# Nilau1998/SAC-Agent

Measured on AMD Instinct MI355X. Metric: env-steps/sec (whole node), boat_env exp-6, 65 536 envs/GPU at 1/2/4/8 MI355X, higher is better.
Workload: dtype f64

## Files before the change

sac-agent_amd/csrc/sacenv_boat.hip:

```cpp

#include <hip/hip_runtime.h>
#include <stdint.h>
#include <string.h>

#include "sacenv.h"

#pragma clang fp contract(off)

namespace {

constexpr int kWave = 64;
constexpr int kMtN = SACENV_MT_N;
constexpr int kMtM = 397;
constexpr uint32_t kMtUpper = 0x80000000u;
constexpr uint32_t kMtLower = 0x7fffffffu;
constexpr uint32_t kMtMatrixA = 0x9908b0dfu;
constexpr int kMaxK = SACENV_MAX_KNOTS;
constexpr int kSlots = SACENV_SLOTS;
constexpr double kPi = 3.141592653589793;

constexpr int U_SX = 0, U_SY = 8, U_SR = 16, U_VX = 24, U_VY = 32, U_VR = 40, U_RUD = 48,
              U_EP = 56, U_COEF = 64, U_W0N = 128, U_T = 144, U_IDX = 152,
              U_CONS = 156, U_FILL = 160, U_MTPOS = 164, U_SYN = 168, U_STARTY = 172,
              U_CNT = U_STARTY + 4 * kSlots,
// ... 320 lines not shown
#pragma unroll
  for (int i = 4; i < 10; ++i) ps = fma_v(ps, z, K.s[i]);
  double pc = fma_v(z, K.c[0], K.c[1]);
#pragma unroll
  for (int i = 2; i < 7; ++i) pc = fma_v(pc, z, K.c[i]);
  sincos_quadrant(r, z, ps, pc, k, sp, cp);
}

__device__ __forceinline__ void sincos_quadrant(double r, double z, double ps, double pc, double k, double* sp,
                                                double* cp) {
  const double sr = fma(r * z, ps, r);
  const double cr = 1.0 - fma(-(z * z), pc, 0.5 * z);
  const int q = (int)k;
  const double a = (q & 1) ? cr : sr, b = (q & 1) ? sr : cr;
  const uint64_t ms = (uint64_t)(((uint32_t)q << 30) & 0x80000000u) << 32;
  const uint64_t mc = (uint64_t)((((uint32_t)q + 1u) << 30) & 0x80000000u) << 32;
  *sp = __longlong_as_double((long long)((uint64_t)__double_as_longlong(a) ^ ms));
  *cp = __longlong_as_double((long long)((uint64_t)__double_as_longlong(b) ^ mc));
}

struct SinCos {
  double s, c;
};
__device__ __forceinline__ double sin_ocml(double x) { return sin(x); }
__device__ __forceinline__ SinCos sincos_ocml(double x) {
  SinCos r;
  sincos(x, &r.s, &r.c);
  return r;
}

__device__ __forceinline__ void sincos_cw(double x, double* sp, double* cp, const TrigK& K) {
  sincos_fast(x, sp, cp, K);
  const bool ok = fabs(x) <= kCwBound;
  if (__ballot(!ok) != 0ull && !ok) {
    const SinCos r = sincos_ocml(x);
    *sp = r.s, *cp = r.c;
  }
}

__device__ __forceinline__ void trig3(double j, double r, double w, double* sj, double* sr, double* sw,
                                      double* cw, const TrigK& K) {
  const double kw = rint(w * 0.6366197723675814);
  double rw = fma(-kw, 1.5707963267948966, w);
  rw = fma(-kw, 6.123233995736766e-17, rw);
  rw = fma(-kw, -1.4973849048591698e-33, rw);
  const double zj = j * j, zr = r * r, zw = rw * rw;
  double qj = fma_v(zj, K.s[0], K.s[1]);
  double qr = fma_v(zr, K.s[0], K.s[1]);
  double ps = 0.0, pc = 0.0;
#pragma unroll
  for (int i = 2; i < 10; ++i) {
    qj = fma_v(qj, zj, K.s[i]);
    qr = fma_v(qr, zr, K.s[i]);
    if (i == 3) ps = fma_v(zw, K.s[2], K.s[3]);
    if (i >= 4) ps = fma_v(ps, zw, K.s[i]);
    if (i == 4) pc = fma_v(zw, K.c[0], K.c[1]);
    if (i >= 5) pc = fma_v(pc, zw, K.c[i - 3]);
  }
  *sj = fma(j * zj, qj, j);
  *sr = fma(r * zr, qr, r);
  sincos_quadrant(rw, zw, ps, pc, kw, sw, cw);
  const bool okj = fabs(j) <= kSinBound, okr = fabs(r) <= kSinBound, okw = fabs(w) <= kCwBound;
  if (__ballot(!(okj && okr && okw)) != 0ull) {
    if (!okj) *sj = sin_ocml(j);
    if (!okr) *sr = sin_ocml(r);
    if (!okw) {
      const SinCos q = sincos_ocml(w);
      *sw = q.s, *cw = q.c;
    }
  }
}

__device__ __forceinline__ double div_c(double x, double c, double r) {
  const double q = x * r;
  const double err = fma(-q, c, x);
  return fma(err, r, q);
}

struct Obs {
  float v[SACENV_OBS_DIM];
};

struct ObsConst {
  double goal, two_w, fuel;
  double k[8];
};

__device__ __forceinline__ ObsConst obs_const(const Tail& T) {
  return ObsConst{T.r_goal, T.r_two_w, T.r_fuel,
                  {1.0 / 5.0, 1.0 / 0.025, 1.0 / 0.37, 1.0 / (2 * kPi), 1.0 / 8.5e-3, 1.0 / 1.4e-5,
                   1.0 / (kPi / 3 - (-kPi / 3)), kPi / 3}};
}
__device__ __forceinline__ ObsConst obs_const_v(const Tail& T) {
  ObsConst o = obs_const(T);
#pragma unroll
  for (int i = 0; i < 8; ++i) o.k[i] = vconst(o.k[i]);
// ... 1097 lines not shown
  int64_t act_stride;
  const uint32_t* ready;
  uint32_t* done;
  uint32_t seq0;
  int32_t* status;
};

__device__ __forceinline__ uint32_t flag_issue(const uint32_t* f) {
  const __amdgpu_buffer_rsrc_t r =
      __builtin_amdgcn_make_buffer_rsrc(const_cast<uint32_t*>(f), 0, 4, 0x00020000);
  return __builtin_amdgcn_raw_buffer_load_b32(r, 0, 0, 17);
}
__device__ __forceinline__ uint32_t flag_value(uint32_t v) {
  return (uint32_t)__builtin_amdgcn_readfirstlane((int)v);
}
__device__ __forceinline__ uint32_t flag_load(const uint32_t* f) { return flag_value(flag_issue(f)); }
__device__ __forceinline__ float act_load(const char* row, uint32_t off) {
  const __amdgpu_buffer_rsrc_t r = __builtin_amdgcn_make_buffer_rsrc(const_cast<char*>(row), 0, 0x7fffffff,
                                                                     0x00020000);
  return __builtin_bit_cast(float, __builtin_amdgcn_raw_buffer_load_b32(r, off, 0, 17));
}
__device__ uint32_t wait_flag(const uint32_t* f, uint32_t want, uint32_t seen, int32_t* status, int lane) {
  for (uint32_t it = 0; seen < want; ++it) {
    if (it >= kSpinLimit) {
      if (lane == 0) atomicOr(status, SACENV_STATUS_HANDOFF_TIMEOUT);
      return 0u;
    }
    __builtin_amdgcn_s_sleep(2);
    seen = flag_load(f);
  }
  return seen;
}

template <bool kRoll, int kNc, bool kTIdx, bool kHand = false, int kRows = 1, bool kVc = kRoll>
__device__ __forceinline__ void owner_wave(const SacenvBoatParams& pin, const Arena& A, const Tail& Tin,
                                           const float* __restrict__ action, OwnerLds& l, int ob,
                                           int lane, int n_steps = 1, const RollArgs* ra = nullptr,
                                           char* trans1 = nullptr, uint32_t seen0 = 0u) {
#ifdef SACENV_STAMPS
  const uint64_t st_real0 = __builtin_amdgcn_s_memrealtime();
  uint64_t st_loaded = 0, st_computed = 0;
#define OWNER_STAMP(v)                                            \
  do {                                                            \
    if (!kRoll) {    \
      asm volatile("s_waitcnt vmcnt(0) lgkmcnt(0)" ::: "memory"); \
      v = __builtin_amdgcn_s_memrealtime();                       \
    }                                                             \
  } while (0)
#else
#define OWNER_STAMP(v) \
  do {                 \
  } while (0)
#endif
  const int e = ob * kWave + lane;
  const uint32_t eo = (uint32_t)e * 8u, eo4 = (uint32_t)e * 4u;
  const char* const wbase = A.wk_wave(ob * kWave);
  const bool active = e < pin.n_envs;
  const char* const abase = reinterpret_cast<const char*>(action) + (active ? eo4 : (uint32_t)ob * 256u);
  uint32_t lt = (uint32_t)A.i32e(U_LTERM, eo4);
  const uint32_t* const rdy = kHand ? (ra->ready != nullptr ? ra->ready + ob : nullptr) : nullptr;
  const int64_t arow = kRoll ? ra->act_stride * 4 : 0;
  uint32_t seen = seen0;
  bool failed = false;
  const bool per_step = kHand && rdy != nullptr && seen < ra->seq0 + (uint32_t)n_steps;
  float act_cur = *reinterpret_cast<const float*>(abase);
  constexpr bool t_idx = kTIdx;
  constexpr int nc = kNc;
  int32_t index = A.i32e(U_IDX, eo4);
  int cons = pin.autoreset ? A.i32e(U_CONS, eo4) : 0;
  double cf[kCoef];
#pragma unroll
  for (int k = 0; k < kCoef; ++k) cf[k] = 0.0;
  if (nc > 0) {
#pragma unroll
    for (int k = 0; k < 4; k += 2) {
      const double2 q = A.f64p(U_COEF + 8 * k, eo);
      cf[k] = q.x, cf[k + 1] = q.y;
    }
    if (nc > 1) {
#pragma unroll
      for (int k = 4; k < 8; k += 2) {
        const double2 q = A.f64p(U_COEF + 8 * k, eo);
        cf[k] = q.x, cf[k + 1] = q.y;
      }
    }
  }
  const double2 p_sxy = A.f64p(U_SX, eo), p_srvx = A.f64p(U_SR, eo), p_vyvr = A.f64p(U_VY, eo);
  const double2 p_rudep = A.f64p(U_RUD, eo);
  double s_x = p_sxy.x, s_y = p_sxy.y, s_r = p_srvx.x;
  double v_x = p_srvx.y, v_y = p_vyvr.x, v_r = p_vyvr.y;
  double rudder = p_rudep.x, t = t_idx ? 0.0 : A.f64e(U_T, eo), ep = p_rudep.y;
  __builtin_amdgcn_sched_barrier(0);
  const SacenvBoatParams& p = pin;
  const Tail& T = Tin;
  constexpr bool kWT = !kRoll || kHand;
  const TrigK K = trig_k<kVc>();
  const ObsConst oc = kVc ? obs_const_v(T) : obs_const(T);
  double y0c[2] = {0.0, 0.0};
  int32_t syc = 0;
  if (kRoll && p.autoreset) {
#pragma unroll
    for (int c = 0; c < 2; ++c)
      if (c < nc) y0c[c] = A.f64e(U_W0N + 8 * c, eo);
    if (p.experiment == 2) syc = A.i32e(U_SYN, eo4);
  }
#ifdef SACENV_STAMPS
  uint64_t ph[4] = {0, 0, 0, 0}, ph_t = 0;
#define PHASE(i)                                         \
  do {                                                   \
    __builtin_amdgcn_sched_barrier(0);                   \
    const uint64_t ph_now = __builtin_amdgcn_s_memtime(); \
    if ((i) > 0) ph[(i) - 1] += ph_now - ph_t;           \
    ph_t = ph_now;                                       \
    __builtin_amdgcn_sched_barrier(0);                   \
  } while (0)
#else
#define PHASE(i) \
  do {           \
  } while (0)
#endif
  Knot kcur = knot_coord(p, index > p.wind_len - 1 ? p.wind_len - 1 : index);
  const uint32_t slot_bytes = 2u * 16u * (uint32_t)A.nk, lane_ring = A.wko_l(0, 0, 0, lane);
  const int slot0 = cons % kSlots;
  int nslot = slot0 + 1 == kSlots ? 0 : slot0 + 1;
  uint32_t so = lane_ring + (uint32_t)slot0 * slot_bytes, sno = lane_ring + (uint32_t)nslot * slot_bytes;
  if (kRoll && kRows == 2) {
    static_assert((kMkWords & (kMkWords - 1)) == 0, "l.mk is indexed (ks / 32) % kMkWords");
    if (ra->marks != nullptr) {
      const int W = (n_steps + 63) / 64;
      unsigned long long* const w = ra->marks + (int64_t)e * W;
      for (int q = 0; q < W; ++q) {
        const unsigned long long m = w[q];
        w[q] = 0ull;
        l.mk[2 * q][lane] = (uint32_t)m;
        l.mk[2 * q + 1][lane] = (uint32_t)(m >> 32);
      }
    } else {
#pragma unroll
      for (int q = 0; q < kMkWords; ++q) l.mk[q][lane] = ~0u;
    }
    __builtin_amdgcn_fence(__ATOMIC_RELEASE, "wavefront");
    __builtin_amdgcn_wave_barrier();
    __builtin_amdgcn_fence(__ATOMIC_ACQUIRE, "wavefront");
  }
  const __amdgpu_buffer_rsrc_t srs = __builtin_amdgcn_make_buffer_rsrc(
      (kRoll && kRows == 2) ? ra->stage + (int64_t)ob * kWave * n_steps * 64 : nullptr, 0, 0x7fffffff, 0x00020000);
  const uint32_t s_lane = (kRoll && kRows == 2) ? (uint32_t)lane * (uint32_t)n_steps * 64u : 0u;
  uint32_t mkw = 0u;
  if (kRoll) __builtin_amdgcn_s_waitcnt(0);
  for (int ks = 0; ks < (kRoll ? n_steps : 1) && (!kHand || !failed); ++ks) {
  PHASE(0);
  const float act = active ? act_cur : 0.0f;
  bool act_next = false;
  uint32_t flag_now = 0u;
  if (kRoll && ks + 1 < n_steps) {
    if (!kHand || !per_step) {
      act_cur = *reinterpret_cast<const float*>(abase + (int64_t)(ks + 1) * arow);
      act_next = true;
    } else {
      if (seen >= ra->seq0 + (uint32_t)ks + 2u) {
        act_cur = act_load(abase, (uint32_t)((ks + 1) * arow));
        act_next = true;
      }
      flag_now = flag_issue(rdy);
    }
  }
  const int wi = index > p.wind_len - 1 ? p.wind_len - 1 : index;
  Knot knext = kcur;
  double wv = 0.0, wa = 0.0;
  bool refresh = false;
  int jn = 0;
  double rq[kCoef];
  if (nc == 0) {
    wind_at(p, A, T.table, 0, e, wi, wv, wa);
  } else {
    const double tt = kcur.t;
    const double c0 = spline_piece(cf[0], cf[2], cf[1], cf[3], tt);
    if (nc == 2) {
      wv = c0;
      wa = spline_piece(cf[4], cf[6], cf[5], cf[7], tt);
    } else if (p.experiment == 4) {
      wv = c0;
      wa = p.wind_dir_rad;
    } else {
      wv = p.max_velocity;
      wa = ((c0 <= 0.5 / 2 ? 0.0 : 1.0) * kPi) + kPi / 2;
    }
    const int wn = index + 1 > p.wind_len - 1 ? p.wind_len - 1 : index + 1;
    knext = knot_coord(p, wn);
    jn = knext.j;
    refresh = index == 0 || jn != kcur.j;
    if (__ballot(refresh) != 0ull) {
#pragma unroll
      for (int c = 0; c < 2; ++c)
        if (c < nc) {
          double q[4];
          A.piece_at(wbase, refresh ? so + (uint32_t)(c * A.nk + jn) * 16u : 0u, q);
          rq[4 * c] = q[0], rq[4 * c + 1] = q[1], rq[4 * c + 2] = q[2], rq[4 * c + 3] = q[3];
        }
    }
  }
  double y0n[2];
  int32_t syn = 0;
  const bool hdr_refresh = p.autoreset && index == 0;
  {
    const int ns = nslot;
#pragma unroll
    for (int c = 0; c < 2; ++c)
      if (c < nc) {
        const double v = *(hdr_refresh ? reinterpret_cast<const double*>(wbase + sno + (uint32_t)(c * A.nk) * 16u)
                                       : (kRoll ? A.wind_knots() : &A.f64e(U_W0N + 8 * c, eo)));
        y0n[c] = kRoll && !hdr_refresh ? y0c[c] : v;
      }
    if (nc == 0 && p.experiment == 2) {
      const int32_t v = *(hdr_refresh ? &A.i32e(U_STARTY + 4 * ns, eo4) : &A.i32e(U_SYN, eo4));
      syn = kRoll && !hdr_refresh ? syc : v;
    }
  }
  OWNER_STAMP(st_loaded);
  const double r_mx = T.r_mx, r_my = T.r_my, r_iz = T.r_iz, r_nd = T.r_nd, r_w = T.r_w;

  t = t_idx ? (double)(index + 1) * p.dt : t + p.dt;
  const int32_t fuel = p.fuel0 - (index + 1);
  if (p.test_mode == 0) rudder = rudder + div_c((double)act, 10.0, 0.1);
  if (!t_idx) EARLY_STORE(U_T, t);
  const bool first = index == 0;
  const double v_x_w = v_x * p.one_minus_wf;
  const double J = p.n_rpm != 0.0 ? div_c(v_x_w, p.n_times_d, r_nd) : 0.0;
  double sin_J, sin_rud, swa, cwa;
  trig3(J, rudder, wa, &sin_J, &sin_rud, &swa, &cwa, K);
  PHASE(1);

  const double F_R = (v_x * v_x) * T.k_front;
  const double F_T = sin_J * T.k_thrust;
  const double F_C = v_y * p.m_plus_my * v_r;
  const double w2s = wv * fabs(wv);
  const double F_W = (w2s * T.k_front) * cwa;
  const double a_x = div_c(-F_R + F_T + F_C + F_W, p.m_plus_mx, r_mx);
  v_x = first ? 3.0 : a_x * p.dt + v_x;

  const double F_R2 = (v_y * fabs(v_y)) * T.k_side;
  const double vx2 = v_x * v_x;
  const double F_RU = sin_rud * (vx2 * T.k_rud_front);
  const double F_C2 = v_x * p.m_plus_mx * v_r;
  const double F_W2 = (w2s * T.k_side) * swa;
  const double a_y = div_c(-F_R2 + F_RU + F_C2 + F_W2, p.m_plus_my, r_my);
  v_y = first ? 0.0 : a_y * p.dt + v_y;
// ... 3 lines not shown
  const double a_r = div_c(-M_hull + M_rud, p.i_plus_iz, r_iz);
  v_r = first ? 0.0 : a_r * p.dt + v_r;
  EARLY_STORE2(U_VY, v_y, v_r);

  s_r = v_r * p.dt + s_r;
  double ssr, csr;
  sincos_cw(s_r, &ssr, &csr, K);
  s_x = (v_x * csr - v_y * ssr) * p.dt + s_x;
  s_y = (v_y * csr + v_x * ssr) * p.dt + s_y;
  index = index + 1;
  EARLY_STORE2(U_SX, s_x, s_y);
  EARLY_STORE2(U_SR, s_r, v_x);
  if (!kRoll) st_out(A.i32e(U_IDX, eo4), index);
  PHASE(2);

  Obs o = make_obs(p, oc, s_x, v_x, a_x, s_y, v_y, a_y, s_r, v_r, a_r, rudder, (double)fuel);

  const double ay = fabs(s_y);
  const double f_y = div_c(ay, p.track_width, r_w) / (1.0 + exp_v(p.reward_k * (ay - p.reward_center), K));
  double reward = 0.0 - f_y;

  const bool goal = s_x >= p.goal_line;
  int tm = (rudder > kPi / 3) | (rudder < -kPi / 3) ? SACENV_TERM_RUDDER_BROKEN : SACENV_TERM_NONE;
  tm = p.t_max <= t ? SACENV_TERM_TIMEOUT : tm;
  tm = fuel < 0 ? SACENV_TERM_OUT_OF_FUEL : tm;
  tm = (fabs(s_y) > p.oob_limit) | (s_x < 0.0) ? SACENV_TERM_OUT_OF_BOUNDS : tm;
  tm = goal ? SACENV_TERM_REACHED_GOAL : tm;
  reward = goal ? reward + 1000.0 : reward;
  reward = ((rudder > kPi / 4) | (rudder < -kPi / 4)) ? reward - fabs(rudder) * 100.0 : reward;
  reward = fabs(s_r) > kPi / 2 ? reward - 1.0 : reward;
  ep = ep + reward;
  uint8_t term = active ? (uint8_t)tm : (uint8_t)SACENV_TERM_NONE;

  if (term != SACENV_TERM_NONE)
    __hip_atomic_fetch_add(&A.at_e<uint32_t>(U_CNT + 4 * (term - 1), eo4), 1u, __ATOMIC_RELAXED,
                           __HIP_MEMORY_SCOPE_AGENT);
  if (term == SACENV_TERM_NONE && active && p.max_episode_steps > 0 && index >= p.max_episode_steps)
    term = SACENV_TERM_TRUNCATED;
  lt = (uint32_t)term - 1u < 5u ? (uint32_t)term : lt;
  const bool ended = term != SACENV_TERM_NONE;
  PHASE(3);

  OWNER_STAMP(st_computed);
  char* const R = kRoll ? ra->rec + (int64_t)ks * ra->rec_stride : A.b + A.ur() * A.np;
  float* const fin = kRoll ? (ra->fin != nullptr ? ra->fin + (int64_t)ks * ra->fin_stride : nullptr)
                           : A.final_obs();
  char* const trans = kRows != 1 ? nullptr
                              : kRoll ? (ra->trans != nullptr ? ra->trans + (int64_t)ks * ra->trans_stride : nullptr)
                                      : trans1;
  if (p.out_flags & SACENV_OUT_REWARD64) A.at_e<double>(A.ur() + 126, eo) = reward;
  if (p.out_flags & SACENV_OUT_ACCEL) {
    A.at_e<double>(A.ur() + 102, eo) = a_x;
    A.at_e<double>(A.ur() + 110, eo) = a_y;
    A.at_e<double>(A.ur() + 118, eo) = a_r;
  }
  const bool restart = ended && p.autoreset;
  if (ended) A.at_e<double>(A.ur() + 94, eo) = ep;
  if (restart && fin != nullptr) store_obs(fin + (int64_t)e * SACENV_OBS_DIM, o);
  int cons_out = cons;
  bool staged = false;
  if (kRoll && kRows == 2) {
    if ((ks & 31) == 0) mkw = l.mk[(ks >> 5) & (kMkWords - 1)][lane];
    staged = (mkw & 1u) != 0u;
    mkw >>= 1;
    if (staged) {
      const uint32_t so = (uint32_t)ks * 64u;
      __builtin_amdgcn_raw_buffer_store_b128(
          u4v{__float_as_uint(o.v[0]), __float_as_uint(o.v[1]), __float_as_uint(o.v[2]), __float_as_uint(o.v[3])},
          srs, s_lane, so, 0);
      __builtin_amdgcn_raw_buffer_store_b128(
          u4v{__float_as_uint(o.v[4]), __float_as_uint(o.v[5]), __float_as_uint(o.v[6]), __float_as_uint(o.v[7])},
          srs, s_lane + 16u, so, 0);
      __builtin_amdgcn_raw_buffer_store_b128(
          u4v{__float_as_uint(o.v[8]), __float_as_uint(o.v[9]), __float_as_uint(o.v[10]), __float_as_uint((float)reward)},
          srs, s_lane + 32u, so, 0);
      __builtin_amdgcn_raw_buffer_store_b128(u4v{__float_as_uint(act), (uint32_t)term | (lt << 8), 0u, 0u}, srs,
                                             s_lane + 48u, so, 0);
    }
  }
  float row[SACENV_OBS_DIM];
#pragma unroll
  for (int k = 0; k < SACENV_OBS_DIM; ++k) row[k] = o.v[k];
  float row3_new = 0.0f;
  const bool any_restart = __ballot(restart) != 0ull;
  if (any_restart) {
    if (restart) {
      const double sy0 = p.experiment == 2 ? (double)syn : 0.0;
      s_x = 0.0, s_y = sy0, s_r = 0.0, v_x = 0.0, v_y = 0.0, v_r = 0.0, rudder = 0.0;
      t = 0.0, ep = 0.0;
      index = 0;
      Obs fo;
      if (p.experiment == 2 || p.fuel0 == 0) {
        fo = make_obs(p, oc, 0.0, 0.0, 0.0, sy0, 0.0, 0.0, 0.0, 0.0, 0.0, 0.0, (double)p.fuel0);
      } else {
        constexpr float kRud0 = (float)((0.0 + kPi / 3) * (1.0 / (kPi / 3 - (-kPi / 3))));
#pragma unroll
        for (int k = 0; k < SACENV_OBS_DIM; ++k) fo.v[k] = 0.0f;
        fo.v[3] = 0.5f;
        fo.v[9] = kRud0;
        fo.v[10] = 1.0f;
      }
#pragma unroll
      for (int k = 0; k < SACENV_OBS_DIM; ++k) row[k] = fo.v[k];
      row3_new = fo.v[3];
      if (kRoll && kRows == 2 && p.experiment == 2 && staged)
        __builtin_amdgcn_raw_buffer_store_b32(__float_as_uint(row3_new), srs, s_lane + 56u, (uint32_t)ks * 64u, 0);
      cons_out = cons + 1;
    }
  }
  if (!kRoll && restart) {
    EARLY_STORE2(U_SX, s_x, s_y);
    EARLY_STORE2(U_SR, s_r, v_x);
    EARLY_STORE2(U_VY, v_y, v_r);
    if (!t_idx) st_out(A.f64e(U_T, eo), t);
    st_out(A.i32e(U_IDX, eo4), index);
    st_out(A.i32e(U_CONS, eo4), cons_out);
  }
  if (!kRoll) {
    st_out(A.i32e(U_LTERM, eo4), (int32_t)lt);
    EARLY_STORE2(U_RUD, rudder, ep);
    if (restart && nc > 0) {
#pragma unroll
      for (int c = 0; c < 2; ++c)
        if (c < nc) st_out(A.f64e(U_COEF + 32 * c, eo), y0n[c]);
    } else if (refresh) {
#pragma unroll
      for (int k = 0; k < kCoef; k += 2)
        if (k < 4 * nc) EARLY_STORE2(U_COEF + 8 * k, rq[k], rq[k + 1]);
    }
    if (hdr_refresh) {
#pragma unroll
      for (int c = 0; c < 2; ++c)
        if (c < nc) st_out(A.f64e(U_W0N + 8 * c, eo), y0n[c]);
      if (p.experiment == 2) st_out(A.i32e(U_SYN, eo4), syn);
    }
  } else {
    if (nc > 0 && __ballot(refresh && !restart) != 0ull && refresh && !restart) {
#pragma unroll
      for (int k = 0; k < kCoef; ++k) cf[k] = rq[k];
    }
#pragma unroll
    for (int c = 0; c < 2; ++c) y0c[c] = y0n[c];
    syc = syn;
    cons = cons_out;
    kcur = knext;
    if (any_restart && restart) {
#pragma unroll
      for (int c = 0; c < 2; ++c)
        if (c < nc) cf[4 * c] = y0n[c];
      so = sno;
      nslot = nslot + 1 == kSlots ? 0 : nslot + 1;
      sno = nslot == 0 ? lane_ring : sno + slot_bytes;
      kcur = knot_coord(p, 0);
    }
  }
  if (kRows == 3) {
    __builtin_nontemporal_store((float)reward, reinterpret_cast<float*>(R + 44 * A.np + eo4));
    __builtin_nontemporal_store((uint8_t)(ended ? 1 : 0), reinterpret_cast<uint8_t*>(R + 48 * A.np + e));
    __builtin_nontemporal_store(term, reinterpret_cast<uint8_t*>(R + 49 * A.np + e));
  } else {
    st_out<kWT>(*reinterpret_cast<float*>(R + 44 * A.np + eo4), (float)reward);
    st_out<kWT>(*reinterpret_cast<uint8_t*>(R + 48 * A.np + e), (uint8_t)(ended ? 1 : 0));
    st_out<kWT>(*reinterpret_cast<uint8_t*>(R + 49 * A.np + e), term);
  }
  if (!kWT) {
    if (kRows == 3)
      store_row_nt<SACENV_OBS_DIM>(reinterpret_cast<float*>(R) + (int64_t)e * SACENV_OBS_DIM, row);
    else
      store_row<SACENV_OBS_DIM>(reinterpret_cast<float*>(R) + (int64_t)e * SACENV_OBS_DIM, row);
  } else {
#pragma unroll
    for (int k = 0; k < SACENV_OBS_DIM; ++k) l.obs[lane * SACENV_OBS_DIM + k] = row[k];
    __builtin_amdgcn_fence(__ATOMIC_RELEASE, "wavefront");
    __builtin_amdgcn_wave_barrier();
    __builtin_amdgcn_fence(__ATOMIC_ACQUIRE, "wavefront");
    const int64_t row0 = (int64_t)ob * kWave * SACENV_OBS_DIM;
    store_obs_block<SACENV_OBS_DIM, kWT>(l.obs, reinterpret_cast<float*>(R) + row0, lane);
    if (kRoll) {
      __builtin_amdgcn_fence(__ATOMIC_RELEASE, "wavefront");
      __builtin_amdgcn_wave_barrier();
      __builtin_amdgcn_fence(__ATOMIC_ACQUIRE, "wavefront");
    }
  }
  if (trans != nullptr) {
    if (!kWT) {
      store_row<SACENV_TRANS_OBS>(reinterpret_cast<float*>(trans) + (int64_t)e * SACENV_TRANS_OBS, o.v);
    } else {
// ... 17 lines not shown
    if (kRoll && kWT) {
      __builtin_amdgcn_fence(__ATOMIC_RELEASE, "wavefront");
      __builtin_amdgcn_wave_barrier();
      __builtin_amdgcn_fence(__ATOMIC_ACQUIRE, "wavefront");
    }
  }
  if (kHand && ra->done != nullptr) {
    __builtin_amdgcn_fence(__ATOMIC_RELEASE, "agent");
    if (lane == 0)
      __hip_atomic_store(ra->done + ob, ra->seq0 + (uint32_t)ks + 1u, __ATOMIC_RELAXED, __HIP_MEMORY_SCOPE_AGENT);
  }
  if (kHand && per_step && ks + 1 < n_steps) {
    const uint32_t fv = flag_value(flag_now);
    seen = fv > seen ? fv : seen;
    failed = seen == SACENV_FLAG_ABORT;
    if (!act_next && !failed) {
      seen = wait_flag(rdy, ra->seq0 + (uint32_t)ks + 2u, seen, ra->status, lane);
      failed = seen == 0u || seen == SACENV_FLAG_ABORT;
      act_cur = act_load(abase, (uint32_t)((ks + 1) * arow));
    }
  }
  PHASE(4);
  }
  if (kHand && failed && ra->done != nullptr && lane == 0)
    __hip_atomic_store(ra->done + ob, SACENV_FLAG_ABORT, __ATOMIC_RELAXED, __HIP_MEMORY_SCOPE_AGENT);
  if (kRoll) {
    A.f64e(U_SX, eo) = s_x, A.f64e(U_SY, eo) = s_y, A.f64e(U_SR, eo) = s_r;
    A.f64e(U_VX, eo) = v_x, A.f64e(U_VY, eo) = v_y, A.f64e(U_VR, eo) = v_r;
    A.f64e(U_RUD, eo) = rudder;
    if (!t_idx) A.f64e(U_T, eo) = t;
    A.f64e(U_EP, eo) = ep;
    A.i32e(U_IDX, eo4) = index;
    A.i32e(U_LTERM, eo4) = (int32_t)lt;
    if (p.autoreset) A.i32e(U_CONS, eo4) = cons;
#pragma unroll
    for (int k = 0; k < kCoef; ++k)
      if (k < 4 * nc) A.f64e(U_COEF + 8 * k, eo) = cf[k];
    if (p.autoreset) {
#pragma unroll
      for (int c = 0; c < 2; ++c)
        if (c < nc) A.f64e(U_W0N + 8 * c, eo) = y0c[c];
      if (p.experiment == 2) A.i32e(U_SYN, eo4) = syc;
    }
  }

#ifdef SACENV_STAMPS
  asm volatile("s_waitcnt vmcnt(0)" ::: "memory");
  if (kRoll && lane == 0) {
    double* d = A.accel() + (int64_t)ob * 8;
    for (int i = 0; i < 4; ++i) d[i] = (double)ph[i];
    d[4] = (double)n_steps;
  } else if (lane == 0) {
    double* d = A.accel() + (int64_t)ob * 4;
    d[0] = (double)st_real0;
    d[1] = (double)__builtin_amdgcn_s_memrealtime();
    d[2] = (double)st_loaded;
    d[3] = (double)st_computed;
  }
#endif
}

template <bool kMixed, int kNc, bool kTIdx>
__global__ void __launch_bounds__(kWave) k_step(SacenvBoatParams p, Arena A, Tail T,
                                                const float* __restrict__ action, int nb_boat,
                                                MixedToys M, char* __restrict__ trans) {
  __shared__ OwnerLds slds;
  const int lane = threadIdx.x;
  int b = (int)blockIdx.x;
  if (!kMixed || b < nb_boat) {
    owner_wave<false, kNc, kTIdx>(p, A, T, action, slds, b, lane, 1, nullptr,
                                  trans);
    return;
  }
  b -= nb_boat;
  if (b < M.nb[0]) {
    toy_wave(M.p[0], M.a[0], b, lane);
  } else if (M.n > 1) {
    toy_wave(M.p[1], M.a[1], b - M.nb[0], lane);
  }
}



template <int kNc, bool kTIdx, int kRows, bool kVc>
__device__ __forceinline__ void rollout_body(const SacenvBoatParams& p, const Arena& A, const Tail& T,
                                             const float* __restrict__ action, int n_steps, const RollArgs& ra,
                                             OwnerLds& slds) {
  const int ob = blockIdx.x, lane = threadIdx.x;
  uint32_t seen = 0u;
  bool hand = ra.done != nullptr;
  if (ra.ready != nullptr || ra.done != nullptr) {
    const uint32_t* rdy = ra.ready != nullptr ? ra.ready + ob : nullptr;
    const uint32_t st = flag_issue(reinterpret_cast<const uint32_t*>(ra.status));
    const uint32_t f0 = rdy != nullptr ? flag_issue(rdy) : 0u;
    bool stop = (flag_value(st) & SACENV_STATUS_HANDOFF_TIMEOUT) != 0u;
    if (!stop && rdy != nullptr) {
      seen = wait_flag(rdy, ra.seq0 + 1u, flag_value(f0), ra.status, lane);
      stop = seen == 0u || seen == SACENV_FLAG_ABORT;
    }
    if (stop) {
      if (ra.done != nullptr && lane == 0)
        __hip_atomic_store(ra.done + ob, SACENV_FLAG_ABORT, __ATOMIC_RELAXED, __HIP_MEMORY_SCOPE_AGENT);
      return;
    }
  }
  if (ra.ready != nullptr) {
    __builtin_amdgcn_fence(__ATOMIC_ACQUIRE, "agent");
    hand = hand || seen < ra.seq0 + (uint32_t)n_steps;
  }
  if (hand) {
    if (kVc)
      owner_wave<true, kNc, kTIdx, true, kRows, true>(vreg_params(p), A, vreg_tail(T), action, slds, ob, lane,
                                                       n_steps, &ra, nullptr, seen);
    else
      owner_wave<true, kNc, kTIdx, true, kRows, false>(p, A, T, action, slds, ob, lane, n_steps, &ra, nullptr, seen);
  } else {
    if (kVc)
      owner_wave<true, kNc, kTIdx, false, kRows, true>(vreg_params(p), A, vreg_tail(T), action, slds, ob, lane,
                                                        n_steps, &ra);
    else
      owner_wave<true, kNc, kTIdx, false, kRows, false>(p, A, T, action, slds, ob, lane, n_steps, &ra);
  }
}
template <int kNc, bool kTIdx, int kRows>
__global__ void __launch_bounds__(kWave) k_rollout(SacenvBoatParams p, Arena A, Tail T,
                                                   const float* __restrict__ action, int n_steps, RollArgs ra) {
  __shared__ OwnerLds slds;
  rollout_body<kNc, kTIdx, kRows, true>(p, A, T, action, n_steps, ra, slds);
}
template <int kNc, bool kTIdx, int kRows>
__global__ void __launch_bounds__(kWave) __attribute__((amdgpu_waves_per_eu(2, 2)))
k_rollout_dense(SacenvBoatParams p, Arena A, Tail T, const float* __restrict__ action, int n_steps, RollArgs ra) {
  __shared__ OwnerLds slds;
  rollout_body<kNc, kTIdx, kRows, false>(p, A, T, action, n_steps, ra, slds);
}

template <int kNc, bool kTIdx>
__global__ void __launch_bounds__(kWave) k_rollout_mixed(SacenvBoatParams p, Arena A, Tail T,
                                                         const float* __restrict__ action, int n_steps, RollArgs ra,
                                                         int nb_boat, MixedToys M) {
  __shared__ OwnerLds slds;
  const int lane = threadIdx.x;
  int b = (int)blockIdx.x;
  if (b < nb_boat) {
    owner_wave<true, kNc, kTIdx, false, 0>(vreg_params(p), A, vreg_tail(T), action, slds, b, lane, n_steps,
                                               &ra);
    return;
  }
  b -= nb_boat;
  if (b < M.nb[0]) {
    toy_roll_wave(M.p[0], M.a[0], b, lane, n_steps);
  } else if (M.n > 1) {
    toy_roll_wave(M.p[1], M.a[1], b - M.nb[0], lane, n_steps);
  }
}

__global__ void __launch_bounds__(kWave) k_toy_init(SacenvToyParams p, ToyArena T, const int32_t* __restrict__ ids,
                                                    int n, int zero_counters) {
  const int q = blockIdx.x * kWave + threadIdx.x;
  if (q >= n) return;
  const int e = ids != nullptr ? ids[q] : q;
  if (e < 0 || e >= p.n_envs) return;
  double f[5];
  float obs[2];
  toy_initial(p, f, obs);
  for (int k = 0; k < 5; ++k) T.f(k)[e] = f[k];
  T.count()[e] = 0;
  if (zero_counters)
    for (int k = 0; k < 3; ++k) T.ctr(k)[e] = 0u;
  reinterpret_cast<float2*>(T.obs())[e] = make_float2(obs[0], obs[1]);
  T.reward()[e] = 0.0f;
  T.done()[e] = 0;
  T.term()[e] = 0;
}

__global__ void __launch_bounds__(kWave) k_toy_step(SacenvToyParams p, ToyArena T) {
  toy_wave(p, T, blockIdx.x, threadIdx.x);
}

// ... 202 lines not shown

static int boat_step(const SacenvBoatParams* p, void* arena, const float* action, char* trans, void* stream) {
  int rc = check_params(p);
  if (rc) return rc;
  if (arena == nullptr || action == nullptr) return SACENV_E_NULL;
  const int nb_boat = (int)(pad64(p->n_envs) / kWave);
#define SACENV_LAUNCH(NC, TI)                                                                         \
  hipLaunchKernelGGL((k_step<false, NC, TI>), dim3(nb_boat), dim3(kWave), 0, (hipStream_t)stream, *p, \
                     make_arena(*p, arena), make_tail(*p, arena), action, nb_boat, MixedToys{}, trans)
  SACENV_OWNER_DISPATCH(*p, SACENV_LAUNCH)
#undef SACENV_LAUNCH
  return launch_status();
}

int sacenv_boat_step(const SacenvBoatParams* p, void* arena, const float* action, void* stream) {
  return boat_step(p, arena, action, nullptr, stream);
}

int sacenv_boat_step_pooled(const SacenvBoatParams* p, void* arena, const float* action, void* trans,
                            void* stream) {
  if (trans == nullptr) return SACENV_E_NULL;
  if ((reinterpret_cast<uintptr_t>(trans) & 15u) != 0u) return SACENV_E_RANGE;
  return boat_step(p, arena, action, static_cast<char*>(trans), stream);
}

static bool dense_grid(int nb_boat) {
  int dev = 0, cus = 0;
  if (hipGetDevice(&dev) != hipSuccess ||
      hipDeviceGetAttribute(&cus, hipDeviceAttributeMultiprocessorCount, dev) != hipSuccess)
    return false;
  return nb_boat > 4 * cus;
}

static int launch_multi(const SacenvBoatParams& p, void* arena, const float* actions, int n_steps, const RollArgs& ra,
                        void* stream) {
  const int nb_boat = (int)(pad64(p.n_envs) / kWave);
  const bool dense = dense_grid(nb_boat);
#define SACENV_LAUNCH_K(KER, NC, TI)                                                                       \
  if (ra.stage != nullptr)                                                                                 \
    hipLaunchKernelGGL((KER<NC, TI, 2>), dim3(nb_boat), dim3(kWave), 0, (hipStream_t)stream, p,            \
                       make_arena(p, arena), make_tail(p, arena), actions, n_steps, ra);                   \
  else if (ra.trans != nullptr)                                                                            \
    hipLaunchKernelGGL((KER<NC, TI, 1>), dim3(nb_boat), dim3(kWave), 0, (hipStream_t)stream, p,            \
                       make_arena(p, arena), make_tail(p, arena), actions, n_steps, ra);                   \
  else if (ra.rec_stride != 0)                                                                             \
    hipLaunchKernelGGL((KER<NC, TI, 3>), dim3(nb_boat), dim3(kWave), 0, (hipStream_t)stream, p,            \
                       make_arena(p, arena), make_tail(p, arena), actions, n_steps, ra);                   \
  else                                                                                                     \
    hipLaunchKernelGGL((KER<NC, TI, 0>), dim3(nb_boat), dim3(kWave), 0, (hipStream_t)stream, p,            \
                       make_arena(p, arena), make_tail(p, arena), actions, n_steps, ra)
#define SACENV_LAUNCH(NC, TI)                  \
  if (dense) {                                 \
    SACENV_LAUNCH_K(k_rollout_dense, NC, TI);  \
  } else {                                     \
    SACENV_LAUNCH_K(k_rollout, NC, TI);        \
  }
  SACENV_OWNER_DISPATCH(p, SACENV_LAUNCH)
#undef SACENV_LAUNCH
#undef SACENV_LAUNCH_K
  return launch_status();
}

static int64_t A_ur_bytes(const SacenvBoatParams& p) {
  SacenvBoatLayout L;
  compute_layout(p.n_envs, p.n_knots, p.wind_len, p.use_wind_table, (p.out_flags & SACENV_OUT_KNOTS) != 0, &L);
  return L.record;
}
static int64_t status_offset(const SacenvBoatParams& p) {
  SacenvBoatLayout L;
  compute_layout(p.n_envs, p.n_knots, p.wind_len, p.use_wind_table, (p.out_flags & SACENV_OUT_KNOTS) != 0, &L);
  return L.status;
}

int sacenv_boat_rollout(const SacenvBoatParams* p, void* arena, const float* actions, int32_t n_steps,
                        void* records, float* final_obs, void* stream) {
  int rc = check_params(p);
  if (rc) return rc;
  if (arena == nullptr || actions == nullptr || records == nullptr) return SACENV_E_NULL;
  if (n_steps < 1 || (p->autoreset && n_steps > SACENV_REFILL_PERIOD)) return SACENV_E_SIZE;
// ... 20 lines not shown
    return SACENV_E_RANGE;
  if (trans != nullptr && ((reinterpret_cast<uintptr_t>(trans) & 15u) != 0u || (trans_stride & 15) != 0))
    return SACENV_E_RANGE;
  if (stage != nullptr && (trans != nullptr || (reinterpret_cast<uintptr_t>(stage) & 15u) != 0u))
    return SACENV_E_RANGE;
  if (stage_marks != nullptr && n_steps > SACENV_REFILL_PERIOD) return SACENV_E_SIZE;
  const Arena A = make_arena(*p, arena);
  RollArgs ra{};
  ra.rec = static_cast<char*>(arena) + A_ur_bytes(*p);
  ra.rec_stride = 0;
  ra.fin = reinterpret_cast<float*>(static_cast<char*>(arena) + A_ur_bytes(*p) + 50 * A.np);
  ra.fin_stride = 0;
  ra.trans = static_cast<char*>(trans);
  ra.trans_stride = trans_stride;
  ra.stage = static_cast<char*>(stage);
  ra.marks = reinterpret_cast<unsigned long long*>(stage_marks);
  ra.act_stride = action_stride;
  ra.ready = act_ready;
  ra.done = step_done;
  ra.seq0 = seq0;
  ra.status = reinterpret_cast<int32_t*>(static_cast<char*>(arena) + status_offset(*p)) + 1;
  return launch_multi(*p, arena, actions, n_steps, ra, stream);
}

int sacenv_boat_segment_occupancy(const SacenvBoatParams* p, int32_t with_trans, int32_t* blocks_per_cu,
                                  int32_t* grid, int32_t* vgprs, int32_t* lds_bytes) {
  int rc = check_params(p);
  if (rc) return rc;
  if (blocks_per_cu == nullptr || grid == nullptr || vgprs == nullptr || lds_bytes == nullptr) return SACENV_E_NULL;
  int nb = 0;
  hipError_t e = hipSuccess;
  hipFuncAttributes fa{};
  const bool dense = dense_grid((int)(pad64(p->n_envs) / kWave));
#define SACENV_OCC_K(KER, NC, TI)                                                                            \
  if (with_trans == 2) {                                                                                     \
    e = hipOccupancyMaxActiveBlocksPerMultiprocessor(&nb, KER<NC, TI, 2>, kWave, 0);                         \
    if (e == hipSuccess) e = hipFuncGetAttributes(&fa, reinterpret_cast<const void*>(KER<NC, TI, 2>));       \
  } else if (with_trans) {                                                                                   \
    e = hipOccupancyMaxActiveBlocksPerMultiprocessor(&nb, KER<NC, TI, 1>, kWave, 0);                         \
    if (e == hipSuccess) e = hipFuncGetAttributes(&fa, reinterpret_cast<const void*>(KER<NC, TI, 1>));       \
  } else {                                                                                                   \
    e = hipOccupancyMaxActiveBlocksPerMultiprocessor(&nb, KER<NC, TI, 0>, kWave, 0);                         \
    if (e == hipSuccess) e = hipFuncGetAttributes(&fa, reinterpret_cast<const void*>(KER<NC, TI, 0>));       \
  }
#define SACENV_OCC(NC, TI)                  \
  if (dense) {                              \
    SACENV_OCC_K(k_rollout_dense, NC, TI);  \
  } else {                                  \
    SACENV_OCC_K(k_rollout, NC, TI);        \
  }
  SACENV_OWNER_DISPATCH(*p, SACENV_OCC)
#undef SACENV_OCC
#undef SACENV_OCC_K
  if (e != hipSuccess) return (int)e;
  *blocks_per_cu = nb;
  *grid = (int32_t)(pad64(p->n_envs) / kWave);
  *vgprs = fa.numRegs;
  *lds_bytes = (int32_t)fa.sharedSizeBytes;
  return SACENV_OK;
}

int sacenv_boat_refill(const SacenvBoatParams* p, void* arena, void* stream) {
  int rc = check_params(p);
  if (rc) return rc;
  if (arena == nullptr) return SACENV_E_NULL;
  if (!p->autoreset) return SACENV_E_MODE;
  const Arena A = make_arena(*p, arena);
  const unsigned mask_blocks = (unsigned)((A.np / kWave + kMaskThreads / kWave - 1) / (kMaskThreads / kWave));
  hipLaunchKernelGGL(k_need_masks, dim3(mask_blocks), dim3(kMaskThreads), 0, (hipStream_t)stream, *p, A);
  if ((rc = launch_status())) return rc;
  hipLaunchKernelGGL(k_refill, dim3(p->n_helpers), dim3(kWave), 0, (hipStream_t)stream, *p, A);
  if ((rc = launch_status())) return rc;
  const int fit_blocks = 8192 + (int)(A.np / kAheadEnvs);
  const Tail T = make_tail(*p, arena);
  if (p->n_knots == 8)
    hipLaunchKernelGGL((k_refill_fit<8, true>), dim3(fit_blocks), dim3(kWave), 0, (hipStream_t)stream, *p, A, T);
  else if (p->n_knots < 8)
    hipLaunchKernelGGL((k_refill_fit<8, false>), dim3(fit_blocks), dim3(kWave), 0, (hipStream_t)stream, *p, A, T);
  else if (p->n_knots == 16)
    hipLaunchKernelGGL((k_refill_fit<16, true>), dim3(fit_blocks), dim3(kWave), 0, (hipStream_t)stream, *p, A, T);
  else
    hipLaunchKernelGGL((k_refill_fit<16, false>), dim3(fit_blocks), dim3(kWave), 0, (hipStream_t)stream, *p, A,
                       T);
  return launch_status();
}

// ... 99 lines not shown
  M.n = n_toys;
  int nb = 0;
  for (int t = 0; t < n_toys; ++t) {
    if ((rc = check_toy(&toy_params[t]))) return rc;
    if (toy_arenas[t] == nullptr) return SACENV_E_NULL;
    M.p[t] = toy_params[t];
    M.a[t] = make_toy_arena(toy_params[t], toy_arenas[t]);
    M.nb[t] = blocks_for(toy_params[t].n_envs, kWave);
    nb += M.nb[t];
  }
  SacenvBoatParams p{};
  Arena A{};
  Tail T{};
  RollArgs ra{};
  int nb_boat = 0;
  if (bp != nullptr) {
    if ((rc = check_params(bp))) return rc;
    if (boat_arena == nullptr || boat_actions == nullptr) return SACENV_E_NULL;
    if (bp->autoreset && n_steps > SACENV_REFILL_PERIOD) return SACENV_E_SIZE;
    if (action_stride < bp->n_envs) return SACENV_E_RANGE;
    p = *bp;
    A = make_arena(p, boat_arena);
    T = make_tail(p, boat_arena);
    ra.rec = static_cast<char*>(boat_arena) + A_ur_bytes(p);
    ra.rec_stride = 0;
    ra.fin = reinterpret_cast<float*>(static_cast<char*>(boat_arena) + A_ur_bytes(p) + 50 * A.np);
    ra.fin_stride = 0;
    ra.act_stride = action_stride;
    ra.status = reinterpret_cast<int32_t*>(static_cast<char*>(boat_arena) + status_offset(p)) + 1;
    nb_boat = (int)(pad64(p.n_envs) / kWave);
    nb += nb_boat;
  }
  if (nb == 0) return SACENV_OK;
#define SACENV_LAUNCH(NC, TI)                                                                                  \
  hipLaunchKernelGGL((k_rollout_mixed<NC, TI>), dim3(nb), dim3(kWave), 0, (hipStream_t)stream, p, A, T,        \
                     boat_actions, n_steps, ra, nb_boat, M)
  SACENV_OWNER_DISPATCH(p, SACENV_LAUNCH)
#undef SACENV_LAUNCH
  return launch_status();
}

int sacenv_boat_wind_eval(const SacenvBoatParams* p, const void* arena, const int32_t* env_ids,
                          const int32_t* idx, int32_t n, double* out_velocity, double* out_angle,
                          void* stream) {
  int rc = check_params(p);
  if (rc) return rc;
  if (!arena || !env_ids || !idx || !out_velocity || !out_angle) return SACENV_E_NULL;
  if (n < 0) return SACENV_E_SIZE;
  if (n == 0) return SACENV_OK;
  void* a = const_cast<void*>(arena);
  hipLaunchKernelGGL(k_wind_eval, dim3(blocks_for(n, 256)), dim3(256), 0, (hipStream_t)stream, *p,
                     make_arena(*p, a), make_tail(*p, a), env_ids, idx, n, out_velocity, out_angle);
  return launch_status();
}

}
```

Baseline: 45.38 billion.

## Add lean specialization for multi-step rollout and move rare episode-end work under ballot

Adds a kLean template variant, selected when out_flags is zero, autoreset is on, the experiment is not 2, fuel is nonzero and strides are zero. In that variant these runtime parameter checks become compile-time constants. In multi-step rollouts, the termination counter atomics, the episode-return store, the final-obs store and the per-restart slot/knot updates now sit inside a wave-uniform branch taken only when some lane ended. The header-refresh loads are also skipped unless some lane needs them. The aim is fewer per-step branches, loads and atomics in the common no-reset case, at the cost of more kernel instantiations and some restructured restart logic that could change semantics subtly.

```diff
diff --git a/sac-agent_amd/csrc/sacenv_boat.hip b/sac-agent_amd/csrc/sacenv_boat.hip
--- a/sac-agent_amd/csrc/sacenv_boat.hip
+++ b/sac-agent_amd/csrc/sacenv_boat.hip
@@ -376,9 +376,11 @@
 __device__ __forceinline__ void sincos_cw(double x, double* sp, double* cp, const TrigK& K) {
   sincos_fast(x, sp, cp, K);
   const bool ok = fabs(x) <= kCwBound;
-  if (__ballot(!ok) != 0ull && !ok) {
-    const SinCos r = sincos_ocml(x);
-    *sp = r.s, *cp = r.c;
+  if (__builtin_expect(__ballot(!ok) != 0ull, 0)) {
+    if (!ok) {
+      const SinCos r = sincos_ocml(x);
+      *sp = r.s, *cp = r.c;
+    }
   }
 }
 
@@ -405,7 +407,7 @@
   *sr = fma(r * zr, qr, r);
   sincos_quadrant(rw, zw, ps, pc, kw, sw, cw);
   const bool okj = fabs(j) <= kSinBound, okr = fabs(r) <= kSinBound, okw = fabs(w) <= kCwBound;
-  if (__ballot(!(okj && okr && okw)) != 0ull) {
+  if (__builtin_expect(__ballot(!(okj && okr && okw)) != 0ull, 0)) {
     if (!okj) *sj = sin_ocml(j);
     if (!okr) *sr = sin_ocml(r);
     if (!okw) {
@@ -1569,7 +1571,7 @@
   return seen;
 }
 
-template <bool kRoll, int kNc, bool kTIdx, bool kHand = false, int kRows = 1, bool kVc = kRoll>
+template <bool kRoll, int kNc, bool kTIdx, bool kHand = false, int kRows = 1, bool kVc = kRoll, bool kLean = false>
 __device__ __forceinline__ void owner_wave(const SacenvBoatParams& pin, const Arena& A, const Tail& Tin,
                                            const float* __restrict__ action, OwnerLds& l, int ob,
                                            int lane, int n_steps = 1, const RollArgs* ra = nullptr,
@@ -1589,6 +1591,11 @@
   do {                 \
   } while (0)
 #endif
+  static_assert(!kLean || kRoll, "the lean options describe a multi-step launch");
+  const bool autoreset = kLean || pin.autoreset != 0;
+  const bool exp2 = !kLean && pin.experiment == 2;
+  const bool no_fuel = !kLean && pin.fuel0 == 0;
+  const uint32_t out_flags = kLean ? 0u : (uint32_t)pin.out_flags;
   const int e = ob * kWave + lane;
   const uint32_t eo = (uint32_t)e * 8u, eo4 = (uint32_t)e * 4u;
   const char* const wbase = A.wk_wave(ob * kWave);
@@ -1604,7 +1611,7 @@
   constexpr bool t_idx = kTIdx;
   constexpr int nc = kNc;
   int32_t index = A.i32e(U_IDX, eo4);
-  int cons = pin.autoreset ? A.i32e(U_CONS, eo4) : 0;
+  int cons = autoreset ? A.i32e(U_CONS, eo4) : 0;
   double cf[kCoef];
 #pragma unroll
   for (int k = 0; k < kCoef; ++k) cf[k] = 0.0;
@@ -1635,11 +1642,11 @@
   const ObsConst oc = kVc ? obs_const_v(T) : obs_const(T);
   double y0c[2] = {0.0, 0.0};
   int32_t syc = 0;
-  if (kRoll && p.autoreset) {
+  if (kRoll && autoreset) {
 #pragma unroll
     for (int c = 0; c < 2; ++c)
       if (c < nc) y0c[c] = A.f64e(U_W0N + 8 * c, eo);
-    if (p.experiment == 2) syc = A.i32e(U_SYN, eo4);
+    if (exp2) syc = A.i32e(U_SYN, eo4);
   }
 #ifdef SACENV_STAMPS
   uint64_t ph[4] = {0, 0, 0, 0}, ph_t = 0;
@@ -1705,7 +1712,7 @@
   const int wi = index > p.wind_len - 1 ? p.wind_len - 1 : index;
   Knot knext = kcur;
   double wv = 0.0, wa = 0.0;
-  bool refresh = false;
+  bool refresh = false, any_refresh = false;
   int jn = 0;
   double rq[kCoef];
   if (nc == 0) {
@@ -1727,7 +1734,8 @@
     knext = knot_coord(p, wn);
     jn = knext.j;
     refresh = index == 0 || jn != kcur.j;
-    if (__ballot(refresh) != 0ull) {
+    any_refresh = __builtin_expect(__ballot(refresh) != 0ull, 0);
+    if (any_refresh) {
 #pragma unroll
       for (int c = 0; c < 2; ++c)
         if (c < nc) {
@@ -1739,8 +1747,11 @@
   }
   double y0n[2];
   int32_t syn = 0;
-  const bool hdr_refresh = p.autoreset && index == 0;
-  {
+  const bool hdr_refresh = autoreset && index == 0;
+#pragma unroll
+  for (int c = 0; c < 2; ++c) y0n[c] = y0c[c];
+  if (kRoll) syn = syc;
+  if (!kRoll || __builtin_expect(__ballot(hdr_refresh) != 0ull, 0)) {
     const int ns = nslot;
 #pragma unroll
     for (int c = 0; c < 2; ++c)
@@ -1749,7 +1760,7 @@
                                        : (kRoll ? A.wind_knots() : &A.f64e(U_W0N + 8 * c, eo)));
         y0n[c] = kRoll && !hdr_refresh ? y0c[c] : v;
       }
-    if (nc == 0 && p.experiment == 2) {
+    if (nc == 0 && exp2) {
       const int32_t v = *(hdr_refresh ? &A.i32e(U_STARTY + 4 * ns, eo4) : &A.i32e(U_SYN, eo4));
       syn = kRoll && !hdr_refresh ? syc : v;
     }
@@ -1819,7 +1830,7 @@
   ep = ep + reward;
   uint8_t term = active ? (uint8_t)tm : (uint8_t)SACENV_TERM_NONE;
 
-  if (term != SACENV_TERM_NONE)
+  if (!kRoll && term != SACENV_TERM_NONE)
     __hip_atomic_fetch_add(&A.at_e<uint32_t>(U_CNT + 4 * (term - 1), eo4), 1u, __ATOMIC_RELAXED,
                            __HIP_MEMORY_SCOPE_AGENT);
   if (term == SACENV_TERM_NONE && active && p.max_episode_steps > 0 && index >= p.max_episode_steps)
@@ -1829,21 +1840,24 @@
   PHASE(3);
 
   OWNER_STAMP(st_computed);
-  char* const R = kRoll ? ra->rec + (int64_t)ks * ra->rec_stride : A.b + A.ur() * A.np;
-  float* const fin = kRoll ? (ra->fin != nullptr ? ra->fin + (int64_t)ks * ra->fin_stride : nullptr)
-                           : A.final_obs();
+  char* const R = kLean ? ra->rec : kRoll ? ra->rec + (int64_t)ks * ra->rec_stride : A.b + A.ur() * A.np;
+  float* const fin = kLean   ? ra->fin
+                     : kRoll ? (ra->fin != nullptr ? ra->fin + (int64_t)ks * ra->fin_stride : nullptr)
+                             : A.final_obs();
   char* const trans = kRows != 1 ? nullptr
                               : kRoll ? (ra->trans != nullptr ? ra->trans + (int64_t)ks * ra->trans_stride : nullptr)
                                       : trans1;
-  if (p.out_flags & SACENV_OUT_REWARD64) A.at_e<double>(A.ur() + 126, eo) = reward;
-  if (p.out_flags & SACENV_OUT_ACCEL) {
+  if (out_flags & SACENV_OUT_REWARD64) A.at_e<double>(A.ur() + 126, eo) = reward;
+  if (out_flags & SACENV_OUT_ACCEL) {
     A.at_e<double>(A.ur() + 102, eo) = a_x;
     A.at_e<double>(A.ur() + 110, eo) = a_y;
     A.at_e<double>(A.ur() + 118, eo) = a_r;
   }
-  const bool restart = ended && p.autoreset;
-  if (ended) A.at_e<double>(A.ur() + 94, eo) = ep;
-  if (restart && fin != nullptr) store_obs(fin + (int64_t)e * SACENV_OBS_DIM, o);
+  const bool restart = ended && autoreset;
+  if (!kRoll) {
+    if (ended) A.at_e<double>(A.ur() + 94, eo) = ep;
+    if (restart && fin != nullptr) store_obs(fin + (int64_t)e * SACENV_OBS_DIM, o);
+  }
   int cons_out = cons;
   bool staged = false;
   if (kRoll && kRows == 2) {
@@ -1869,15 +1883,21 @@
 #pragma unroll
   for (int k = 0; k < SACENV_OBS_DIM; ++k) row[k] = o.v[k];
   float row3_new = 0.0f;
-  const bool any_restart = __ballot(restart) != 0ull;
-  if (any_restart) {
+  if (kRoll ? __builtin_expect(__ballot(ended) != 0ull, 0) : __ballot(restart) != 0ull) {
+    if (kRoll) {
+      if ((uint32_t)term - 1u < 5u)
+        __hip_atomic_fetch_add(&A.at_e<uint32_t>(U_CNT + 4 * (term - 1), eo4), 1u, __ATOMIC_RELAXED,
+                               __HIP_MEMORY_SCOPE_AGENT);
+      if (ended) A.at_e<double>(A.ur() + 94, eo) = ep;
+      if (restart && fin != nullptr) store_obs(fin + (int64_t)e * SACENV_OBS_DIM, o);
+    }
     if (restart) {
-      const double sy0 = p.experiment == 2 ? (double)syn : 0.0;
+      const double sy0 = exp2 ? (double)syn : 0.0;
       s_x = 0.0, s_y = sy0, s_r = 0.0, v_x = 0.0, v_y = 0.0, v_r = 0.0, rudder = 0.0;
       t = 0.0, ep = 0.0;
       index = 0;
       Obs fo;
-      if (p.experiment == 2 || p.fuel0 == 0) {
+      if (exp2 || no_fuel) {
         fo = make_obs(p, oc, 0.0, 0.0, 0.0, sy0, 0.0, 0.0, 0.0, 0.0, 0.0, 0.0, (double)p.fuel0);
       } else {
         constexpr float kRud0 = (float)((0.0 + kPi / 3) * (1.0 / (kPi / 3 - (-kPi / 3))));
@@ -1890,9 +1910,18 @@
 #pragma unroll
       for (int k = 0; k < SACENV_OBS_DIM; ++k) row[k] = fo.v[k];
       row3_new = fo.v[3];
-      if (kRoll && kRows == 2 && p.experiment == 2 && staged)
+      if (kRoll && kRows == 2 && exp2 && staged)
         __builtin_amdgcn_raw_buffer_store_b32(__float_as_uint(row3_new), srs, s_lane + 56u, (uint32_t)ks * 64u, 0);
       cons_out = cons + 1;
+      if (kRoll) {
+#pragma unroll
+        for (int c = 0; c < 2; ++c)
+          if (c < nc) cf[4 * c] = y0n[c];
+        so = sno;
+        nslot = nslot + 1 == kSlots ? 0 : nslot + 1;
+        sno = nslot == 0 ? lane_ring : sno + slot_bytes;
+        knext = knot_coord(p, 0);
+      }
     }
   }
   if (!kRoll && restart) {
@@ -1919,27 +1948,20 @@
 #pragma unroll
       for (int c = 0; c < 2; ++c)
         if (c < nc) st_out(A.f64e(U_W0N + 8 * c, eo), y0n[c]);
-      if (p.experiment == 2) st_out(A.i32e(U_SYN, eo4), syn);
+      if (exp2) st_out(A.i32e(U_SYN, eo4), syn);
     }
   } else {
-    if (nc > 0 && __ballot(refresh && !restart) != 0ull && refresh && !restart) {
-#pragma unroll
-      for (int k = 0; k < kCoef; ++k) cf[k] = rq[k];
+    if (nc > 0 && any_refresh) {
+      if (refresh && !restart) {
+#pragma unroll
+        for (int k = 0; k < kCoef; ++k) cf[k] = rq[k];
+      }
     }
 #pragma unroll
     for (int c = 0; c < 2; ++c) y0c[c] = y0n[c];
     syc = syn;
     cons = cons_out;
     kcur = knext;
-    if (any_restart && restart) {
-#pragma unroll
-      for (int c = 0; c < 2; ++c)
-        if (c < nc) cf[4 * c] = y0n[c];
-      so = sno;
-      nslot = nslot + 1 == kSlots ? 0 : nslot + 1;
-      sno = nslot == 0 ? lane_ring : sno + slot_bytes;
-      kcur = knot_coord(p, 0);
-    }
   }
   if (kRows == 3) {
     __builtin_nontemporal_store((float)reward, reinterpret_cast<float*>(R + 44 * A.np + eo4));
@@ -2023,15 +2045,15 @@
     A.f64e(U_EP, eo) = ep;
     A.i32e(U_IDX, eo4) = index;
     A.i32e(U_LTERM, eo4) = (int32_t)lt;
-    if (p.autoreset) A.i32e(U_CONS, eo4) = cons;
+    if (autoreset) A.i32e(U_CONS, eo4) = cons;
 #pragma unroll
     for (int k = 0; k < kCoef; ++k)
       if (k < 4 * nc) A.f64e(U_COEF + 8 * k, eo) = cf[k];
-    if (p.autoreset) {
+    if (autoreset) {
 #pragma unroll
       for (int c = 0; c < 2; ++c)
         if (c < nc) A.f64e(U_W0N + 8 * c, eo) = y0c[c];
-      if (p.experiment == 2) A.i32e(U_SYN, eo4) = syc;
+      if (exp2) A.i32e(U_SYN, eo4) = syc;
     }
   }
 
@@ -2073,7 +2095,7 @@
 
 
 
-template <int kNc, bool kTIdx, int kRows, bool kVc>
+template <int kNc, bool kTIdx, int kRows, bool kVc, bool kLean>
 __device__ __forceinline__ void rollout_body(const SacenvBoatParams& p, const Arena& A, const Tail& T,
                                              const float* __restrict__ action, int n_steps, const RollArgs& ra,
                                              OwnerLds& slds) {
@@ -2107,26 +2129,26 @@
       owner_wave<true, kNc, kTIdx, true, kRows, false>(p, A, T, action, slds, ob, lane, n_steps, &ra, nullptr, seen);
   } else {
     if (kVc)
-      owner_wave<true, kNc, kTIdx, false, kRows, true>(vreg_params(p), A, vreg_tail(T), action, slds, ob, lane,
-                                                        n_steps, &ra);
+      owner_wave<true, kNc, kTIdx, false, kRows, true, kLean>(vreg_params(p), A, vreg_tail(T), action, slds, ob,
+                                                               lane, n_steps, &ra);
     else
-      owner_wave<true, kNc, kTIdx, false, kRows, false>(p, A, T, action, slds, ob, lane, n_steps, &ra);
-  }
-}
-template <int kNc, bool kTIdx, int kRows>
+      owner_wave<true, kNc, kTIdx, false, kRows, false, kLean>(p, A, T, action, slds, ob, lane, n_steps, &ra);
+  }
+}
+template <int kNc, bool kTIdx, int kRows, bool kLean = false>
 __global__ void __launch_bounds__(kWave) k_rollout(SacenvBoatParams p, Arena A, Tail T,
                                                    const float* __restrict__ action, int n_steps, RollArgs ra) {
   __shared__ OwnerLds slds;
-  rollout_body<kNc, kTIdx, kRows, true>(p, A, T, action, n_steps, ra, slds);
-}
-template <int kNc, bool kTIdx, int kRows>
+  rollout_body<kNc, kTIdx, kRows, true, kLean>(p, A, T, action, n_steps, ra, slds);
+}
+template <int kNc, bool kTIdx, int kRows, bool kLean = false>
 __global__ void __launch_bounds__(kWave) __attribute__((amdgpu_waves_per_eu(2, 2)))
 k_rollout_dense(SacenvBoatParams p, Arena A, Tail T, const float* __restrict__ action, int n_steps, RollArgs ra) {
   __shared__ OwnerLds slds;
-  rollout_body<kNc, kTIdx, kRows, false>(p, A, T, action, n_steps, ra, slds);
-}
-
-template <int kNc, bool kTIdx>
+  rollout_body<kNc, kTIdx, kRows, false, kLean>(p, A, T, action, n_steps, ra, slds);
+}
+
+template <int kNc, bool kTIdx, bool kLean = false>
 __global__ void __launch_bounds__(kWave) k_rollout_mixed(SacenvBoatParams p, Arena A, Tail T,
                                                          const float* __restrict__ action, int n_steps, RollArgs ra,
                                                          int nb_boat, MixedToys M) {
@@ -2134,8 +2156,8 @@
   const int lane = threadIdx.x;
   int b = (int)blockIdx.x;
   if (b < nb_boat) {
-    owner_wave<true, kNc, kTIdx, false, 0>(vreg_params(p), A, vreg_tail(T), action, slds, b, lane, n_steps,
-                                               &ra);
+    owner_wave<true, kNc, kTIdx, false, 0, true, kLean>(vreg_params(p), A, vreg_tail(T), action, slds, b, lane,
+                                                         n_steps, &ra);
     return;
   }
   b -= nb_boat;
@@ -2404,12 +2426,21 @@
   return nb_boat > 4 * cus;
 }
 
+static bool lean_launch(const SacenvBoatParams& p, const RollArgs& ra) {
+  return p.out_flags == 0 && p.autoreset != 0 && p.experiment != 2 && p.fuel0 != 0 && ra.rec_stride == 0 &&
+         ra.fin_stride == 0;
+}
+
 static int launch_multi(const SacenvBoatParams& p, void* arena, const float* actions, int n_steps, const RollArgs& ra,
                         void* stream) {
   const int nb_boat = (int)(pad64(p.n_envs) / kWave);
   const bool dense = dense_grid(nb_boat);
+  const bool lean = lean_launch(p, ra);
 #define SACENV_LAUNCH_K(KER, NC, TI)                                                                       \
-  if (ra.stage != nullptr)                                                                                 \
+  if (ra.stage != nullptr && lean)                                                                         \
+    hipLaunchKernelGGL((KER<NC, TI, 2, true>), dim3(nb_boat), dim3(kWave), 0, (hipStream_t)stream, p,      \
+                       make_arena(p, arena), make_tail(p, arena), actions, n_steps, ra);                   \
+  else if (ra.stage != nullptr)                                                                            \
     hipLaunchKernelGGL((KER<NC, TI, 2>), dim3(nb_boat), dim3(kWave), 0, (hipStream_t)stream, p,            \
                        make_arena(p, arena), make_tail(p, arena), actions, n_steps, ra);                   \
   else if (ra.trans != nullptr)                                                                            \
@@ -2417,6 +2448,9 @@
                        make_arena(p, arena), make_tail(p, arena), actions, n_steps, ra);                   \
   else if (ra.rec_stride != 0)                                                                             \
     hipLaunchKernelGGL((KER<NC, TI, 3>), dim3(nb_boat), dim3(kWave), 0, (hipStream_t)stream, p,            \
+                       make_arena(p, arena), make_tail(p, arena), actions, n_steps, ra);                   \
+  else if (lean)                                                                                           \
+    hipLaunchKernelGGL((KER<NC, TI, 0, true>), dim3(nb_boat), dim3(kWave), 0, (hipStream_t)stream, p,      \
                        make_arena(p, arena), make_tail(p, arena), actions, n_steps, ra);                   \
   else                                                                                                     \
     hipLaunchKernelGGL((KER<NC, TI, 0>), dim3(nb_boat), dim3(kWave), 0, (hipStream_t)stream, p,            \
@@ -2503,8 +2537,16 @@
   hipError_t e = hipSuccess;
   hipFuncAttributes fa{};
   const bool dense = dense_grid((int)(pad64(p->n_envs) / kWave));
+  const bool lean = lean_launch(*p, RollArgs{});
+#define SACENV_OCC_ONE(K)                                                        \
+  e = hipOccupancyMaxActiveBlocksPerMultiprocessor(&nb, K, kWave, 0);            \
+  if (e == hipSuccess) e = hipFuncGetAttributes(&fa, reinterpret_cast<const void*>(K))
 #define SACENV_OCC_K(KER, NC, TI)                                                                            \
-  if (with_trans == 2) {                                                                                     \
+  if (with_trans == 2 && lean) {                                                                             \
+    SACENV_OCC_ONE((KER<NC, TI, 2, true>));                                                                  \
+  } else if (with_trans == 0 && lean) {                                                                      \
+    SACENV_OCC_ONE((KER<NC, TI, 0, true>));                                                                  \
+  } else if (with_trans == 2) {                                                                              \
     e = hipOccupancyMaxActiveBlocksPerMultiprocessor(&nb, KER<NC, TI, 2>, kWave, 0);                         \
     if (e == hipSuccess) e = hipFuncGetAttributes(&fa, reinterpret_cast<const void*>(KER<NC, TI, 2>));       \
   } else if (with_trans) {                                                                                   \
@@ -2523,6 +2565,7 @@
   SACENV_OWNER_DISPATCH(*p, SACENV_OCC)
 #undef SACENV_OCC
 #undef SACENV_OCC_K
+#undef SACENV_OCC_ONE
   if (e != hipSuccess) return (int)e;
   *blocks_per_cu = nb;
   *grid = (int32_t)(pad64(p->n_envs) / kWave);
@@ -2688,9 +2731,14 @@
     nb += nb_boat;
   }
   if (nb == 0) return SACENV_OK;
+  const bool lean = lean_launch(p, ra);
 #define SACENV_LAUNCH(NC, TI)                                                                                  \
-  hipLaunchKernelGGL((k_rollout_mixed<NC, TI>), dim3(nb), dim3(kWave), 0, (hipStream_t)stream, p, A, T,        \
-                     boat_actions, n_steps, ra, nb_boat, M)
+  if (lean)                                                                                                    \
+    hipLaunchKernelGGL((k_rollout_mixed<NC, TI, true>), dim3(nb), dim3(kWave), 0, (hipStream_t)stream, p, A,   \
+                       T, boat_actions, n_steps, ra, nb_boat, M);                                              \
+  else                                                                                                         \
+    hipLaunchKernelGGL((k_rollout_mixed<NC, TI>), dim3(nb), dim3(kWave), 0, (hipStream_t)stream, p, A, T,      \
+                       boat_actions, n_steps, ra, nb_boat, M)
   SACENV_OWNER_DISPATCH(p, SACENV_LAUNCH)
 #undef SACENV_LAUNCH
   return launch_status();
```

Result: faster. 49.63 billion (median of 6 runs) (+9.4%).
